# OpenGVLab/VisionLLM

Hardware: NVIDIA H100
Metric: img_text_pairs_per_sec_fwd_1024px_256tok (higher is better)
Workload: dtype bf16

## Files before the change

include/vllm_b200.h:

```cpp
#ifndef VLLM_B200_H
#define VLLM_B200_H
#include <stdint.h>
#include <stddef.h>
#ifdef __cplusplus
extern "C" {
#endif

#define VLLM_OK 0
#define VLLM_EINVAL (-1)
#define VLLM_EUNSUPPORTED (-2)
#define VLLM_EALIGN (-3)

const char* vllm_version(void);

#define VLLM_MSDA_STRICT 1
int vllm_msda_forward_f32(const float* value, const int64_t* spatial_shapes, const int64_t* level_start_index,
                          const float* sampling_loc, const float* attn_weight, float* out, int batch,
                          int spatial_size, int num_heads, int channels, int num_levels, int num_query,
                          int num_point, const int64_t* host_shapes_hint, int flags, void* stream);
int vllm_msda_forward_bf16v(const void* value, const int64_t* spatial_shapes, const int64_t* level_start_index,
                            const float* sampling_loc, const float* attn_weight, void* out, int out_bf16, int batch,
                            int spatial_size, int num_heads, int channels, int num_levels, int num_query,
                            int num_point, const int64_t* host_shapes_hint, void* stream);
int vllm_msda_forward_f64(const double* value, const int64_t* spatial_shapes, const int64_t* level_start_index,
// ... 24 lines not shown
                                 int spatial_size, int num_heads, int channels, int num_levels, int num_query, int num_point,
                                 const int64_t* host_shapes_hint, void* stream);

int vllm_dcnv3_forward_f32(const float* input, const float* offset, const float* mask, float* out, int N,
                           int H_in, int W_in, int H_out, int W_out, int group, int group_channels,
                           int kernel_h, int kernel_w, int stride_h, int stride_w, int pad_h, int pad_w,
                           int dilation_h, int dilation_w, float offset_scale, int flags, void* stream);

int vllm_dcnv3_backward_f32(const float* input, const float* offset, const float* mask, const float* grad_output,
                            float* grad_input, float* grad_offset, float* grad_mask, int N, int H_in, int W_in,
                            int H_out, int W_out, int group, int group_channels, int kernel_h, int kernel_w,
                            int stride_h, int stride_w, int pad_h, int pad_w, int dilation_h, int dilation_w,
                            float offset_scale, void* stream);

#define VLLM_ACT_NONE 0
#define VLLM_ACT_GELU 1
#define VLLM_ACT_RELU 2
#define VLLM_ACT_SILU 3
#define VLLM_ACT_SWIGLU 4
#define VLLM_ACT_QUICKGELU 5
int vllm_gemm_bf16(const void* A, int lda, const void* B, int ldb, void* C, int ldc, int M, int N, int K,
                   const void* bias, const void* colscale, const void* residual, int ldr, int act, int out_f32,
                   void* stream);
int vllm_gemm_bf16_rowmask(const void* A, int lda, const void* B, int ldb, void* C, int ldc, int M, int N, int K,
                           const void* bias, const void* colscale, const void* residual, int ldr, int act, int out_f32,
                           const unsigned char* row_keep, void* stream);
int vllm_gemm_set_sm_limit(int all_gemms, int scatter_gemm);
int vllm_conv_rows_bf16(const void* xpad, long long pad_pixels, int channels, int padded_width, int kernel_h,
                        int kernel_w, const void* weight, int ldw, void* out, int ldo, int out_channels,
                        const void* bias, int act, void* stream);
#define VLLM_GEMM_DEFAULT 0
#define VLLM_GEMM_WIDE_TILE 2
#define VLLM_GEMM_NARROW_TILE 3
int vllm_gemm_set_variant(int variant);

int vllm_rmsnorm_bf16(const void* x, long long ldx, const void* weight, void* y, long long ldy, long long rows,
                      int cols, float eps, void* stream);
int vllm_layernorm_bf16(const void* x, long long ldx, const void* weight, const void* bias, void* y, long long ldy,
                        long long rows, int cols, float eps, void* stream);
int vllm_layernorm_gelu_bf16(const void* x, long long ldx, const void* weight, const void* bias, void* y,
                             long long ldy, long long rows, int cols, float eps, void* stream);
int vllm_layernorm_gather_bf16(const void* x, long long ldx, const int64_t* index, long long rows_in, long long rows_out,
                               long long batch, const void* weight, const void* bias, void* y, long long ldy, int cols,
                               float eps, void* stream);
int vllm_layernorm_residual_bf16(const void* x, long long ldx, const void* weight, const void* bias,
                                 const void* residual, long long ldr, void* y, long long ldy, long long rows, int cols,
                                 float eps, void* stream);
int vllm_dcnv3_prep_f32(const void* packed, long long ld, void* offset, void* mask, void* scale, long long rows,
                        int group, int taps, void* stream);
int vllm_dcnv3_blend_bf16(const void* core, const void* xproj, const void* scale, void* out, long long rows,
                          int channels, int group_channels, void* stream);
int vllm_dwconv_nhwc_bf16(const void* x, const void* weight_taps, const void* bias, void* y, int batch, int height,
                          int width, int channels, int kernel, void* stream);
long long vllm_groupnorm_workspace_bytes(int batch, int groups);
int vllm_groupnorm_nhwc_bf16_grid(const void* x, void* y, const void* gamma, const void* beta, int batch, long long h, long long w,
                                  long long x_w_pitch, long long x_image_pitch, int channels, int groups, float eps, int relu,
                                  void* workspace, long long workspace_bytes, void* stream);
int vllm_upsample_add_nhwc_bf16_ex(const void* top, long long top_image_pitch, const void* lateral, void* out, int batch, int in_h,
                                   int in_w, int out_h, int out_w, int channels, int out_pad, void* stream);
int vllm_rope_bf16(void* x, long long ld, const void* cos, const void* sin, long long tokens, int heads,
                   int head_dim, void* stream);

int vllm_attention_bf16(const void* q, const void* k, const void* v, void* o, int batch, int Tq, int Tk,
                        int heads, int kv_heads, int head_dim, long long q_batch_pitch,
                        long long q_token_pitch, long long k_batch_pitch, long long k_token_pitch,
                        long long v_batch_pitch, long long v_token_pitch, long long o_batch_pitch,
// ... 91 lines not shown
```

visionllm_b200/_lib.py:

```python
import contextlib
import ctypes
import os
import threading

_HERE = os.path.dirname(os.path.abspath(__file__))
LIB_PATH = os.path.join(_HERE, "lib", "libvllm_b200.so")

_lock = threading.Lock()
_lib = None
_launches = 0

c_i64p = ctypes.POINTER(ctypes.c_int64)
vp = ctypes.c_void_p
ci = ctypes.c_int
cll = ctypes.c_longlong
cf = ctypes.c_float

_SIGNATURES = {
    "vllm_version": (ctypes.c_char_p, []),
    "vllm_msda_forward_f32": (ci, [vp, vp, vp, vp, vp, vp, ci, ci, ci, ci, ci, ci, ci, vp, ci, vp]),
    "vllm_msda_forward_bf16v": (ci, [vp, vp, vp, vp, vp, vp, ci, ci, ci, ci, ci, ci, ci, ci, vp, vp]),
    "vllm_msda_forward_f64": (ci, [vp, vp, vp, vp, vp, vp, ci, ci, ci, ci, ci, ci, ci, vp]),
    "vllm_msda_backward_f32": (ci, [vp] * 9 + [ci] * 7 + [vp]),
    "vllm_msda_backward_f64": (ci, [vp] * 9 + [ci] * 7 + [vp]),
# ... 35 lines not shown
    "vllm_layernorm_bf16": (ci, [vp, cll, vp, vp, vp, cll, cll, ci, cf, vp]),
    "vllm_layernorm_gelu_bf16": (ci, [vp, cll, vp, vp, vp, cll, cll, ci, cf, vp]),
    "vllm_layernorm_gather_bf16": (ci, [vp, cll, vp, cll, cll, cll, vp, vp, vp, cll, ci, cf, vp]),
    "vllm_layernorm_residual_bf16": (ci, [vp, cll, vp, vp, vp, cll, vp, cll, cll, ci, cf, vp]),
    "vllm_dcnv3_prep_f32": (ci, [vp, cll, vp, vp, vp, cll, ci, ci, vp]),
    "vllm_dcnv3_blend_bf16": (ci, [vp, vp, vp, vp, cll, ci, ci, vp]),
    "vllm_dwconv_nhwc_bf16": (ci, [vp, vp, vp, vp, ci, ci, ci, ci, ci, vp]),
    "vllm_rope_bf16": (ci, [vp, cll, vp, vp, cll, ci, ci, vp]),
    "vllm_groupnorm_workspace_bytes": (cll, [ci, ci]),
    "vllm_upsample_add_nhwc_bf16_ex": (ci, [vp, cll, vp, vp, ci, ci, ci, ci, ci, ci, ci, vp]),
    "vllm_groupnorm_nhwc_bf16_grid": (ci, [vp, vp, vp, vp, ci, cll, cll, cll, cll, ci, ci, cf, ci, vp, cll, vp]),
    "vllm_attention_bf16": (ci, [vp, vp, vp, vp, ci, ci, ci, ci, ci, ci, cll, cll, cll, cll, cll, cll, cll, cll,
                                 vp, vp, vp, vp, ci, ci, cf, vp, cll, vp]),
    "vllm_attention_bf16_tiles": (ci, [vp, vp, vp, vp, ci, ci, ci, ci, ci, ci, cll, cll, cll, cll, cll, cll, cll, cll,
                                       vp, vp, vp, cf, vp, vp, vp]),
    "vllm_attention_mask_tiles": (ci, [vp, cll, ci, ci, vp, vp, vp]),
    "vllm_attention_set_variant": (ci, [ci]),
    "vllm_attention_set_splits": (ci, [ci]),
    "vllm_peer_alloc": (ci, [ctypes.POINTER(vp), ctypes.c_size_t]),
    "vllm_peer_free": (ci, [vp]),
    "vllm_peer_handle_bytes": (ci, []),
    "vllm_peer_export": (ci, [vp, vp]),
    "vllm_peer_open": (ci, [vp, ctypes.POINTER(vp)]),
    "vllm_peer_close": (ci, [vp]),
    "vllm_gemm_bf16_scatter": (ci, [vp, ci, vp, ci, vp, vp, ci, ci, ci, ci, ci, vp]),
    "vllm_tp_reduce_norm_bf16": (ci, [vp, ci, cll, vp, vp, cf, vp, ci, cll, vp, ctypes.c_uint, vp, ci, ci, ci, vp]),
    "vllm_tp_norm_ctas": (ci, [ci]),
    "vllm_tp_wait": (ci, [vp, ctypes.c_uint, vp]),
    "vllm_tp_signal": (ci, [vp, ci, ctypes.c_uint, vp]),
}


MSDA_DEFAULT, MSDA_NO_HINT, MSDA_BF16_NO_WINDOW, MSDA_FP32_WINDOW = 0, 4, 32, 33
GEMM_DEFAULT, GEMM_WIDE_TILE, GEMM_NARROW_TILE = 0, 2, 3
ATTN_DEFAULT, ATTN_WARP_MMA = 0, 1

_KNOB_DEFAULTS = {"msda_set_variant": (MSDA_DEFAULT,), "msda_set_window": (0, 0, 0), "msda_set_window_fill": (-1,),
                  "gemm_set_variant": (GEMM_DEFAULT,), "gemm_set_sm_limit": (0, 0), "attention_set_variant": (ATTN_DEFAULT,),
                  "attention_set_splits": (0,)}


class VllmB200Error(RuntimeError):
    pass


def exported_symbols():
    return sorted(_SIGNATURES)


def lib():
    global _lib
    if _lib is None:
        with _lock:
            if _lib is None:
                if not os.path.exists(LIB_PATH):
                    raise ImportError(
                        f"{LIB_PATH} is missing: build it with `make` or "
                        "`python -c 'import __graft_entry__ as g; g.build()'`. "
                        "visionllm_b200 has no CPU/eager fallback.")
                L = ctypes.CDLL(LIB_PATH)
                for name, (res, args) in _SIGNATURES.items():
                    fn = getattr(L, name)
                    fn.restype = res
                    fn.argtypes = args
                _lib = L
    return _lib

# ... 34 lines not shown
```

visionllm_b200/csrc/gemm.cu:

```cuda
#include "common.cuh"
#include "tc_common.cuh"
#include "vllm_b200.h"

namespace {

constexpr int BM = 128, BK = 64, THREADS = 384, CONSUMER_WARPS = 8, CONSUMER_THREADS = CONSUMER_WARPS * 32;
constexpr int A_BYTES = BM * BK * 2;
constexpr int EPI_BUF = 16 * 128;
constexpr int SMEM_LIMIT = 232448;

enum { ACT_NONE = 0, ACT_GELU = 1, ACT_RELU = 2, ACT_SILU = 3, ACT_SWIGLU = 4, ACT_QUICKGELU = 5 };

struct GemmArgs {
  int M, N, K;
  void* C; int ldc;
  const __nv_bfloat16* bias; const __nv_bfloat16* colscale; const __nv_bfloat16* residual; int ldr;
  int act; int out_f32;
  const unsigned char* row_keep;
  int tiles_m, tiles_n;
  int group_m;
  int a_seg_kb, a_seg_rows;
  int sc_rows;
  void* sc_dst[8];
  uint32_t* sc_flag[8];
  int a_mn, b_mn;
  int bt_rows, causal;
  int group, reduce;
};

struct TilePlan { int skip, kb0, kb1, segs, b_row_off, a_k_off, b_k_off; };
__device__ __forceinline__ TilePlan plan_tile(const GemmArgs& g, int m0, int n0, int rows_per_tile, int num_kb) {
  TilePlan p{0, 0, num_kb, 1, 0, 0, 0};
  if (g.bt_rows) {
    const int bh = m0 / g.bt_rows, ml = m0 - bh * g.bt_rows;
    const int a_mat = g.reduce ? bh * g.group : bh;
    const int b_mat = g.reduce ? bh * g.group : bh / g.group;
    p.segs = g.reduce ? g.group : 1;
    p.b_row_off = b_mat * g.N;
    p.a_k_off = a_mat * g.K;
    p.b_k_off = b_mat * g.K;
    if (g.causal == 1 && n0 >= ml + rows_per_tile) p.skip = 1;
    if (g.causal == 2) p.kb0 = ml / BK;
    if (g.causal == 3) { const int e = (ml + rows_per_tile + BK - 1) / BK; p.kb1 = e < num_kb ? e : num_kb; }
  }
  return p;
}

template <int BN> struct Cfg {
  static constexpr int B_BYTES = BN * BK * 2;
  static constexpr int STAGE_BYTES = A_BYTES + B_BYTES;
  static constexpr int STAGES = BN == 256 ? 4 : 6;
  static constexpr int EPI_OFF = STAGES * STAGE_BYTES;
  static constexpr int BAR_OFF = EPI_OFF + CONSUMER_WARPS * 2 * EPI_BUF;
  static constexpr int BIAS_OFF = BAR_OFF + 256;
  static constexpr int SCALE_OFF = BIAS_OFF + 2 * BN + 4;
  static constexpr int KEEP_OFF = SCALE_OFF + 2 * BN + 4;
  static constexpr int SMEM = 1024  + KEEP_OFF + BM + 4;
  static_assert(8 * (2 * STAGES + 2 * CONSUMER_WARPS) <= 256, "mbarriers overflow their slot");
  static_assert(SMEM <= SMEM_LIMIT, "shared memory over the per-block limit");
};

__device__ __forceinline__ float gelu_erf(float x) { return 0.5f * x * (1.f + erff(x * 0.70710678118654752f)); }
__device__ __forceinline__ float silu(float x) { return x / (1.f + __expf(-x)); }

__device__ __forceinline__ void tile_coords(int t, int tiles_m, int tiles_n, int group_m, int& tm, int& tn) {
  const int per_group = group_m * tiles_n;
  const int group = t / per_group;
  const int first = group * group_m;
  const int gsz = min(group_m, tiles_m - first);
  const int in = t - group * per_group;
  tm = first + in % gsz;
  tn = in / gsz;
}

template <int BN, int TA, int TB>
__device__ __forceinline__ void mma_kblock(float (&acc)[BN / 2], uint32_t sa, uint32_t sb, bool first_kb) {
  const uint64_t adesc = TA ? tc::wgmma_desc_sw128(sa, 8192, 1024) : tc::wgmma_desc_sw128(sa, 16, 1024);
  const uint64_t bdesc = TB ? tc::wgmma_desc_sw128(sb, 8192, 1024) : tc::wgmma_desc_sw128(sb, 16, 1024);
  constexpr uint64_t astep = TA ? 128 : 2, bstep = TB ? 128 : 2;
#pragma unroll
  for (int k = 0; k < BK / 16; ++k) {
    if constexpr (BN == 256)
      tc::wgmma_m64n256k16_ss<TA, TB>(acc, adesc + astep * k, bdesc + bstep * k, !(first_kb && k == 0));
    else
      tc::wgmma_m64n128k16_ss<TA, TB>(acc, adesc + astep * k, bdesc + bstep * k, !(first_kb && k == 0));
  }
}

enum { EPI_BF16 = 0, EPI_SWIGLU = 1, EPI_F32 = 2, EPI_SCATTER = 3 };

__device__ __forceinline__ int swz(int r, int b) { return r * 128 + ((((b >> 4) ^ r) & 7) << 4) + (b & 15); }

template <int BN, int TA, int TB, int EPI>
__global__ void __launch_bounds__(THREADS, 1)
gemm_bf16_wgmma_kernel(const __grid_constant__ CUtensorMap tmap_a, const __grid_constant__ CUtensorMap tmap_b,
                       const __grid_constant__ CUtensorMap tmap_c, const __grid_constant__ CUtensorMap tmap_r,
                       const GemmArgs g) {
  using C_ = Cfg<BN>;
  constexpr int STAGES = C_::STAGES;
  extern __shared__ uint8_t smem_raw[];
  const uint32_t smem_base = (tc::smem_u32(smem_raw) + 1023u) & ~1023u;
  uint8_t* smem_gen = smem_raw + (smem_base - tc::smem_u32(smem_raw));
  const uint32_t bar_base = smem_base + C_::BAR_OFF;
  auto full_bar = [&](int s) { return bar_base + 8 * s; };
  auto empty_bar = [&](int s) { return bar_base + 8 * (STAGES + s); };
  auto res_bar = [&](int i) { return bar_base + 8 * (2 * STAGES + i); };

  const int warp = threadIdx.x >> 5, lane = threadIdx.x & 31;
  const int n_tiles = g.tiles_m * g.tiles_n;
  const int num_kb = (g.K + BK - 1) / BK;

  if (warp == 0 && lane == 0) {
    tc::tma_prefetch_desc(&tmap_a);
    tc::tma_prefetch_desc(&tmap_b);
    if constexpr (EPI != EPI_SCATTER) {
      tc::tma_prefetch_desc(&tmap_c);
      if (g.residual) tc::tma_prefetch_desc(&tmap_r);
    }
  }
  if (warp == 1 && lane == 0) {
    for (int s = 0; s < STAGES; ++s) { tc::mbar_init(full_bar(s), 1); tc::mbar_init(empty_bar(s), CONSUMER_WARPS); }
    for (int i = 0; i < 2 * CONSUMER_WARPS; ++i) tc::mbar_init(res_bar(i), 1);
    tc::mbar_fence_init();
  }
  __syncthreads();

  if (warp < 4) {
    tc::reg_dealloc<40>();
    if (warp == 0 && tc::elect_one()) {
      int stage = 0; uint32_t phase = 0;
      for (int t = blockIdx.x; t < n_tiles; t += gridDim.x) {
        int tm, tn; tile_coords(t, g.tiles_m, g.tiles_n, g.group_m, tm, tn);
        const TilePlan tp = plan_tile(g, tm * BM, tn * BN, BM, num_kb);
        if (tp.skip) continue;
        const int bt_m0 = g.bt_rows ? (tm * BM) / g.bt_rows * g.bt_rows : 0;
        const int row_a = tm * BM - (TA ? bt_m0 : 0);
        const int row_b = tn * BN + (TB ? 0 : tp.b_row_off);
        for (int gs = 0; gs < tp.segs; ++gs) {
          const int ka_off = TA ? tp.a_k_off + gs * g.K : 0, kb_off = TB ? tp.b_k_off + gs * g.K : 0;
          for (int kb = tp.kb0; kb < tp.kb1; ++kb) {
            tc::mbar_wait(empty_bar(stage), phase ^ 1);
            const uint32_t sa = smem_base + stage * C_::STAGE_BYTES, sb = sa + A_BYTES;
            int ka = kb * BK + ka_off, ra = row_a;
            if (g.a_seg_kb) {
              const int seg = kb / g.a_seg_kb;
              ka = (kb - seg * g.a_seg_kb) * BK;
              ra = row_a + seg * g.a_seg_rows;
            }
            tc::mbar_arrive_expect_tx(full_bar(stage), C_::STAGE_BYTES);
            if constexpr (TA) {
              for (int h = 0; h < BM / 64; ++h) tc::tma_load_2d(sa + h * 8192, &tmap_a, full_bar(stage), ra + 64 * h, ka);
            } else {
              tc::tma_load_2d(sa, &tmap_a, full_bar(stage), ka, ra);
            }
            if constexpr (TB) {
              for (int h = 0; h < BN / 64; ++h)
                tc::tma_load_2d(sb + h * 8192, &tmap_b, full_bar(stage), row_b + 64 * h, kb * BK + kb_off);
            } else {
              tc::tma_load_2d(sb, &tmap_b, full_bar(stage), kb * BK, row_b);
            }
            if (++stage == STAGES) { stage = 0; phase ^= 1; }
          }
        }
      }
    }
    return;
  }

  tc::reg_alloc<232>();
  const int wg = (warp - 4) >> 2;
  const int cw = warp - 4;
  const int et = threadIdx.x - 128;
  const int lr = lane >> 2, frag_col = 2 * (lane & 3);
  const bool has_res = EPI != EPI_SCATTER && g.residual != nullptr;
  constexpr int UNIT_COLS = EPI == EPI_SWIGLU ? 128 : 64;
  constexpr int UNITS = BN / UNIT_COLS;
  constexpr int RES_AHEAD = EPI == EPI_F32 ? 1 : 2;
  const int n_out = EPI == EPI_SWIGLU ? g.N / 2 : g.N;
  uint8_t* s_buf = smem_gen + C_::EPI_OFF + cw * 2 * EPI_BUF;
  const uint32_t s_buf_u32 = smem_base + C_::EPI_OFF + cw * 2 * EPI_BUF;
  const uint32_t s_bias = smem_base + C_::BIAS_OFF, s_scale = smem_base + C_::SCALE_OFF, s_keep = smem_base + C_::KEEP_OFF;
  const __nv_bfloat16* bias_t = reinterpret_cast<const __nv_bfloat16*>(smem_gen + C_::BIAS_OFF + (reinterpret_cast<uintptr_t>(g.bias) & 3));
  const __nv_bfloat16* scale_t =
      reinterpret_cast<const __nv_bfloat16*>(smem_gen + C_::SCALE_OFF + (reinterpret_cast<uintptr_t>(g.colscale) & 3));
  const uint8_t* keep_t = smem_gen + C_::KEEP_OFF + (reinterpret_cast<uintptr_t>(g.row_keep) & 3);
  if (et <= BN / 2) {
    if (!g.bias) *reinterpret_cast<uint32_t*>(smem_gen + C_::BIAS_OFF + 4 * et) = 0u;
    if (!g.colscale) *reinterpret_cast<uint32_t*>(smem_gen + C_::SCALE_OFF + 4 * et) = 0x3F803F80u;
  }
  uint32_t res_phase = 0;
  int stage = 0; uint32_t phase = 0;
  float acc[BN / 2];
  for (int t = blockIdx.x; t < n_tiles; t += gridDim.x) {
    int tm, tn; tile_coords(t, g.tiles_m, g.tiles_n, g.group_m, tm, tn);
    const TilePlan tp = plan_tile(g, tm * BM, tn * BN, BM, num_kb);
    if (tp.skip) continue;
    const int n0 = tn * BN;
    const int oc0 = EPI == EPI_SWIGLU ? n0 / 2 : n0;
    const int warp_row0 = tm * BM + cw * 16;
    const bool warp_live = warp_row0 < g.M;
    if (g.bias && et <= BN / 2) tc::cp_async_vec_word(s_bias, g.bias, 2LL * g.N, 2LL * n0, et);
    if (g.colscale && et <= BN / 2) tc::cp_async_vec_word(s_scale, g.colscale, 2LL * g.N, 2LL * n0, et);
    if (g.row_keep && et <= BM / 4) tc::cp_async_vec_word(s_keep, g.row_keep, g.M, (long long)tm * BM, et);
    auto load_res = [&](int u) {
      const int b = EPI == EPI_F32 ? 0 : (u & 1);
      tc::mbar_arrive_expect_tx(res_bar(2 * cw + b), EPI_BUF);
      tc::tma_load_2d(s_buf_u32 + b * EPI_BUF, &tmap_r, res_bar(2 * cw + b), oc0 + 64 * u, warp_row0);
    };
    if (has_res && warp_live && lane == 0) {
      tc::bulk_wait_read<0>();
#pragma unroll
      for (int u = 0; u < RES_AHEAD && u < UNITS; ++u)
        if (oc0 + 64 * u < n_out) load_res(u);
    }
    int prev_stage = -1;
    const int n_kb = tp.segs * (tp.kb1 - tp.kb0);
    for (int kb = 0; kb < n_kb; ++kb) {
      tc::mbar_wait(full_bar(stage), phase);
      const uint32_t sa = smem_base + stage * C_::STAGE_BYTES + wg * 8192, sb = smem_base + stage * C_::STAGE_BYTES + A_BYTES;
      const bool first = kb == 0;
      tc::acc_fence(acc);
      tc::wgmma_fence();
      mma_kblock<BN, TA, TB>(acc, sa, sb, first);
      tc::wgmma_commit();
      tc::wgmma_wait<1>();
      if (prev_stage >= 0 && lane == 0) tc::mbar_arrive(empty_bar(prev_stage));
      prev_stage = stage;
      if (++stage == STAGES) { stage = 0; phase ^= 1; }
    }
    tc::wgmma_wait<0>();
    tc::acc_fence(acc);
    if (lane == 0) tc::mbar_arrive(empty_bar(prev_stage));
    tc::cp_async_wait_all();
    tc::named_bar_sync(1, CONSUMER_THREADS);

#pragma unroll
    for (int j = 0; j < BN / 8; ++j) {
      const int c = 8 * j + frag_col;
      const float b0 = __bfloat162float(bias_t[c]), b1 = __bfloat162float(bias_t[c + 1]);
      acc[4 * j] = __fadd_rn(acc[4 * j], b0); acc[4 * j + 1] = __fadd_rn(acc[4 * j + 1], b1);
      acc[4 * j + 2] = __fadd_rn(acc[4 * j + 2], b0); acc[4 * j + 3] = __fadd_rn(acc[4 * j + 3], b1);
    }
    if constexpr (EPI == EPI_BF16 || EPI == EPI_F32) {
      switch (g.act) {
        case ACT_GELU:
#pragma unroll
          for (int i = 0; i < BN / 2; ++i) acc[i] = gelu_erf(acc[i]);
          break;
        case ACT_RELU:
#pragma unroll
          for (int i = 0; i < BN / 2; ++i) acc[i] = fmaxf(acc[i], 0.f);
          break;
        case ACT_SILU:
#pragma unroll
          for (int i = 0; i < BN / 2; ++i) acc[i] = silu(acc[i]);
          break;
        case ACT_QUICKGELU:
#pragma unroll
          for (int i = 0; i < BN / 2; ++i) acc[i] = acc[i] / (1.f + __expf(-1.702f * acc[i]));
          break;
        default: break;
      }
    }
    bool keep0 = true, keep1 = true;
    if (g.row_keep) { keep0 = keep_t[cw * 16 + lr] != 0; keep1 = keep_t[cw * 16 + lr + 8] != 0; }

    constexpr int E = EPI == EPI_F32 ? 4 : 2;
    auto put_box = [&](int bi, int col0) {
      if ((n_out * E) % 16 == 0 || col0 + 128 / E <= n_out) {
        if (lane == 0) tc::tma_store_2d(&tmap_c, s_buf_u32 + bi * EPI_BUF, col0, warp_row0);
        return;
      }
#pragma unroll
      for (int it = 0; it < 4; ++it) {
        const int rr = it * 4 + (lane >> 3), piece = lane & 7, row = warp_row0 + rr;
        if (row >= g.M) continue;
#pragma unroll
        for (int e = 0; e < 16 / E; ++e) {
          const int col = col0 + piece * (16 / E) + e;
          if (col >= n_out) break;
          const uint8_t* sp = s_buf + bi * EPI_BUF + swz(rr, 16 * piece + E * e);
          uint8_t* dp = reinterpret_cast<uint8_t*>(g.C) + ((size_t)row * g.ldc + col) * E;
          if constexpr (E == 4) *reinterpret_cast<uint32_t*>(dp) = *reinterpret_cast<const uint32_t*>(sp);
          else *reinterpret_cast<uint16_t*>(dp) = *reinterpret_cast<const uint16_t*>(sp);
        }
      }
    };

    if (warp_live) {
#pragma unroll
      for (int u = 0; u < UNITS; ++u) {
        if (oc0 + 64 * u >= n_out) break;
        const int b = EPI == EPI_F32 ? 0 : (u & 1);
        uint8_t* buf = s_buf + b * EPI_BUF;
        if (has_res) {
          if (u > 0 && u + RES_AHEAD - 1 < UNITS && oc0 + 64 * (u + RES_AHEAD - 1) < n_out && lane == 0) {
            tc::bulk_wait_read<0>();
            load_res(u + RES_AHEAD - 1);
          }
          tc::mbar_wait(res_bar(2 * cw + b), (res_phase >> b) & 1);
          res_phase ^= 1u << b;
        } else if constexpr (EPI != EPI_SCATTER && EPI != EPI_F32) {
          if (lane == 0) { if (u == 0) tc::bulk_wait_read<0>(); else tc::bulk_wait_read<1>(); }
          __syncwarp();
        }
        if constexpr (EPI == EPI_SWIGLU) {
#pragma unroll
          for (int jj = 0; jj < 16; ++jj) {
            const int j = 16 * u + jj;
#pragma unroll
            for (int h = 0; h < 2; ++h) {
              uint8_t* p = buf + swz(lr + 8 * h, 16 * (jj >> 1)) + 8 * (jj & 1) + 2 * (lane & 3);
              float o = __fmul_rn(silu(acc[4 * j + 2 * h]), acc[4 * j + 2 * h + 1]);
              if (has_res) o = __fadd_rn(o, __bfloat162float(*reinterpret_cast<const __nv_bfloat16*>(p)));
              *reinterpret_cast<__nv_bfloat16*>(p) = __float2bfloat16(o);
            }
          }
        } else {
#pragma unroll
          for (int jj = 0; jj < 8; ++jj) {
            const int j = 8 * u + jj, c = 8 * j + frag_col;
            const float s0 = __bfloat162float(scale_t[c]), s1 = __bfloat162float(scale_t[c + 1]);
#pragma unroll
            for (int h = 0; h < 2; ++h) {
              float& v0 = acc[4 * j + 2 * h];
              float& v1 = acc[4 * j + 2 * h + 1];
              uint8_t* p = buf + swz(lr + 8 * h, 16 * jj) + 4 * (lane & 3);
              v0 = __fmul_rn(v0, s0); v1 = __fmul_rn(v1, s1);
              if (has_res) {
                const float2 f = __bfloat1622float2(*reinterpret_cast<const __nv_bfloat162*>(p));
                v0 = __fadd_rn(v0, f.x); v1 = __fadd_rn(v1, f.y);
              }
              if (!(h ? keep1 : keep0)) { v0 = 0.f; v1 = 0.f; }
              if constexpr (EPI != EPI_F32) *reinterpret_cast<__nv_bfloat162*>(p) = __floats2bfloat162_rn(v0, v1);
            }
          }
          if constexpr (EPI == EPI_F32) {
            if (lane == 0) tc::bulk_wait_read<0>();
            __syncwarp();
#pragma unroll
            for (int jj = 0; jj < 8; ++jj) {
              const int j = 8 * u + jj;
#pragma unroll
              for (int h = 0; h < 2; ++h) {
                uint8_t* p = s_buf + (jj >> 2) * EPI_BUF + swz(lr + 8 * h, 32 * (jj & 3) + 8 * (lane & 3));
                *reinterpret_cast<float2*>(p) = make_float2(acc[4 * j + 2 * h], acc[4 * j + 2 * h + 1]);
              }
            }
          }
        }
        if constexpr (EPI == EPI_SCATTER) {
          __syncwarp();
          const int d = warp_row0 / g.sc_rows;
          __nv_bfloat16* dst = reinterpret_cast<__nv_bfloat16*>(g.sc_dst[d]) + (size_t)(warp_row0 - d * g.sc_rows) * g.ldc + n0 + 64 * u;
#pragma unroll
          for (int it = 0; it < 4; ++it) {
            const int rr = it * 4 + (lane >> 3), piece = lane & 7;
            const uint4 val = *reinterpret_cast<const uint4*>(buf + swz(rr, 16 * piece));
            *reinterpret_cast<uint4*>(dst + (size_t)rr * g.ldc + piece * 8) = val;
          }
          __syncwarp();
        } else {
          tc::fence_proxy_async_smem();
          __syncwarp();
          if constexpr (EPI == EPI_F32) {
            put_box(0, n0 + 64 * u);
            if (n0 + 64 * u + 32 < n_out) put_box(1, n0 + 64 * u + 32);
          } else {
            put_box(b, oc0 + 64 * u);
          }
          if (lane == 0) tc::bulk_commit();
        }
      }
    }
    if constexpr (EPI == EPI_SCATTER) {
      __threadfence_system();
      __syncwarp();
      if (lane == 0 && warp_live)
        asm volatile("red.release.sys.global.add.u32 [%0], %1;" ::"l"(g.sc_flag[warp_row0 / g.sc_rows]), "r"(1u) : "memory");
    }
    tc::named_bar_sync(1, CONSUMER_THREADS);
  }
  if (EPI != EPI_SCATTER && lane == 0) tc::bulk_wait<0>();
}

int g_sm_limit = 0, g_scatter_sm_limit = 0;

int g_gemm_variant = VLLM_GEMM_DEFAULT;

using KernelFn = void (*)(const CUtensorMap, const CUtensorMap, const CUtensorMap, const CUtensorMap, const GemmArgs);

template <int BN, int TA, int TB>
KernelFn pick_epilogue(const GemmArgs& g) {
  if (g.sc_rows) {
    if constexpr (BN == 256 && !TA && !TB) return gemm_bf16_wgmma_kernel<BN, TA, TB, EPI_SCATTER>;
    return nullptr;
  }
  if (g.act == ACT_SWIGLU) {
    if constexpr (!TA && !TB) return gemm_bf16_wgmma_kernel<BN, TA, TB, EPI_SWIGLU>;
    return nullptr;
  }
  if (g.out_f32) return gemm_bf16_wgmma_kernel<BN, TA, TB, EPI_F32>;
  return gemm_bf16_wgmma_kernel<BN, TA, TB, EPI_BF16>;
}
template <int BN>
KernelFn pick_kernel(const GemmArgs& g) {
  if (g.a_mn) return g.b_mn ? pick_epilogue<BN, 1, 1>(g) : pick_epilogue<BN, 1, 0>(g);
  return g.b_mn ? pick_epilogue<BN, 0, 1>(g) : pick_epilogue<BN, 0, 0>(g);
}

template <int BN>
int launch_gemm(const void* A, int lda, const void* B, int ldb, GemmArgs g, cudaStream_t st, long long a_rows = -1,
                int a_cols = -1) {
  using C_ = Cfg<BN>;
  CUtensorMap ta, tb;
  const uint64_t nb = g.bt_rows ? (uint64_t)(g.M / g.bt_rows) : 1;
  const uint64_t na = g.bt_rows && g.reduce ? nb * g.group : nb;
  const uint64_t nbb = !g.bt_rows ? 1 : g.reduce ? nb * g.group : nb / g.group;
  const uint64_t m_local = g.bt_rows ? (uint64_t)g.bt_rows : (uint64_t)g.M;
  int rc = g.a_mn ? vllm_make_tmap_2d(&ta, A, na * (uint64_t)g.K, m_local, (uint64_t)lda, 64)
                  : vllm_make_tmap_2d(&ta, A, (uint64_t)(a_rows < 0 ? g.M : a_rows),
                                        (uint64_t)(a_cols < 0 ? g.K : a_cols), (uint64_t)lda, BM);
  if (rc) return rc;
  rc = g.b_mn ? vllm_make_tmap_2d(&tb, B, nbb * (uint64_t)g.K, (uint64_t)g.N, (uint64_t)ldb, 64)
              : vllm_make_tmap_2d(&tb, B, nbb * (uint64_t)g.N, (uint64_t)g.K, (uint64_t)ldb, BN);
  if (rc) return rc;
  CUtensorMap tc_{}, tr{};
  if (!g.sc_rows) {
    const uint64_t n_out = (uint64_t)(g.act == ACT_SWIGLU ? g.N / 2 : g.N);
    rc = vllm_make_tmap_2d(&tc_, g.C, (uint64_t)g.M, n_out, (uint64_t)g.ldc, 16, g.out_f32 != 0);
    if (!rc && g.residual) rc = vllm_make_tmap_2d(&tr, g.residual, (uint64_t)g.M, n_out, (uint64_t)g.ldr, 16);
    if (rc) return rc;
  }
  g.tiles_m = (g.M + BM - 1) / BM;
  g.tiles_n = (g.N + BN - 1) / BN;
  const int n_tiles = g.tiles_m * g.tiles_n;
  int sms = vllm_num_sms();
  const int limit = g.sc_rows ? (g_scatter_sm_limit > 0 ? g_scatter_sm_limit : g_sm_limit) : g_sm_limit;
  if (limit > 0 && limit < sms) sms = limit;
  const int ctas = sms < n_tiles ? sms : n_tiles;
  g.group_m = 8;
  const KernelFn kern = pick_kernel<BN>(g);
  if (!kern) return VLLM_EUNSUPPORTED;
  const cudaError_t e = vllm_smem_optin(kern, C_::SMEM);
  if (e != cudaSuccess) return (int)e;
  kern<<<ctas, THREADS, C_::SMEM, st>>>(ta, tb, tc_, tr, g);
  VLLM_CHECK_LAUNCH();
  return VLLM_OK;
}

bool wide_by_shape(const GemmArgs& g) {
  return !g.a_mn && !g.b_mn && !g.bt_rows && !g.a_seg_kb && g.N >= 2048;
}

int launch_gemm_auto(const void* A, int lda, const void* B, int ldb, const GemmArgs& g, cudaStream_t st, long long a_rows = -1,
                     int a_cols = -1) {
  const bool wide = g.sc_rows || g_gemm_variant == VLLM_GEMM_WIDE_TILE ||
                    (g_gemm_variant == VLLM_GEMM_DEFAULT && wide_by_shape(g));
  return wide ? launch_gemm<256>(A, lda, B, ldb, g, st, a_rows, a_cols) : launch_gemm<128>(A, lda, B, ldb, g, st, a_rows, a_cols);
}

}

extern "C" {

int vllm_gemm_set_variant(int v) {
  if (v != VLLM_GEMM_DEFAULT && v != VLLM_GEMM_WIDE_TILE && v != VLLM_GEMM_NARROW_TILE) return VLLM_EINVAL;
  g_gemm_variant = v;
  return VLLM_OK;
}
int vllm_gemm_set_sm_limit(int all_gemms, int scatter_gemm) {
  if (all_gemms < 0 || scatter_gemm < 0) return VLLM_EINVAL;
  g_sm_limit = all_gemms; g_scatter_sm_limit = scatter_gemm;
  return VLLM_OK;
}

static int gemm_bf16_common(const void* A, int lda, const void* B, int ldb, void* C, int ldc, int M, int N, int K,
                            const void* bias, const void* colscale, const void* residual, int ldr, int act, int out_f32,
                            const unsigned char* row_keep, void* stream);

int vllm_gemm_bf16(const void* A, int lda, const void* B, int ldb, void* C, int ldc, int M, int N, int K,
                   const void* bias, const void* colscale, const void* residual, int ldr, int act, int out_f32,
                   void* stream) {
  return gemm_bf16_common(A, lda, B, ldb, C, ldc, M, N, K, bias, colscale, residual, ldr, act, out_f32, nullptr, stream);
}

int vllm_gemm_bf16_rowmask(const void* A, int lda, const void* B, int ldb, void* C, int ldc, int M, int N, int K,
                           const void* bias, const void* colscale, const void* residual, int ldr, int act, int out_f32,
                           const unsigned char* row_keep, void* stream) {
  if (!row_keep || act == ACT_SWIGLU) return VLLM_EINVAL;
  return gemm_bf16_common(A, lda, B, ldb, C, ldc, M, N, K, bias, colscale, residual, ldr, act, out_f32, row_keep, stream);
}

static int gemm_bf16_common(const void* A, int lda, const void* B, int ldb, void* C, int ldc, int M, int N, int K,
                            const void* bias, const void* colscale, const void* residual, int ldr, int act, int out_f32,
                            const unsigned char* row_keep, void* stream) {
  if (M < 0 || N <= 0 || K <= 0 || lda < K || ldb < K) return VLLM_EINVAL;
  if (M == 0) return VLLM_OK;
  if (!A || !B || !C) return VLLM_EINVAL;
  if (act < 0 || act > ACT_QUICKGELU) return VLLM_EINVAL;
// ... 104 lines not shown
```

Baseline: 6.995.

## Add opt-in ping-pong GEMM schedule and widen tile raster group

Adds a ping-pong variant of the WGMMA GEMM kernel. Each consumer warpgroup computes a full 128x128 tile on its own, using two 64-row accumulators, and the two warpgroups alternate mainloops through ordering mbarriers so one group's epilogue overlaps the other's MMAs. Bias, scale and row-keep vectors are duplicated per warpgroup. The variant only runs when selected explicitly, but the raster group size rises from 8 to 16 for every GEMM, which changes L2 reuse patterns.

```diff
diff --git a/include/vllm_b200.h b/include/vllm_b200.h
--- a/include/vllm_b200.h
+++ b/include/vllm_b200.h
@@ -80,6 +80,7 @@
 #define VLLM_GEMM_DEFAULT 0
 #define VLLM_GEMM_WIDE_TILE 2
 #define VLLM_GEMM_NARROW_TILE 3
+#define VLLM_GEMM_PINGPONG 4
 int vllm_gemm_set_variant(int variant);
 
 int vllm_rmsnorm_bf16(const void* x, long long ldx, const void* weight, void* y, long long ldy, long long rows,
diff --git a/visionllm_b200/_lib.py b/visionllm_b200/_lib.py
--- a/visionllm_b200/_lib.py
+++ b/visionllm_b200/_lib.py
@@ -91,7 +91,7 @@
 
 
 MSDA_DEFAULT, MSDA_NO_HINT, MSDA_BF16_NO_WINDOW, MSDA_FP32_WINDOW = 0, 4, 32, 33
-GEMM_DEFAULT, GEMM_WIDE_TILE, GEMM_NARROW_TILE = 0, 2, 3
+GEMM_DEFAULT, GEMM_WIDE_TILE, GEMM_NARROW_TILE, GEMM_PINGPONG = 0, 2, 3, 4
 ATTN_DEFAULT, ATTN_WARP_MMA = 0, 1
 
 _KNOB_DEFAULTS = {"msda_set_variant": (MSDA_DEFAULT,), "msda_set_window": (0, 0, 0), "msda_set_window_fill": (-1,),
diff --git a/visionllm_b200/csrc/gemm.cu b/visionllm_b200/csrc/gemm.cu
--- a/visionllm_b200/csrc/gemm.cu
+++ b/visionllm_b200/csrc/gemm.cu
@@ -46,7 +46,7 @@
   return p;
 }
 
-template <int BN> struct Cfg {
+template <int BN, bool PINGPONG = false> struct Cfg {
   static constexpr int B_BYTES = BN * BK * 2;
   static constexpr int STAGE_BYTES = A_BYTES + B_BYTES;
   static constexpr int STAGES = BN == 256 ? 4 : 6;
@@ -55,8 +55,11 @@
   static constexpr int BIAS_OFF = BAR_OFF + 256;
   static constexpr int SCALE_OFF = BIAS_OFF + 2 * BN + 4;
   static constexpr int KEEP_OFF = SCALE_OFF + 2 * BN + 4;
-  static constexpr int SMEM = 1024  + KEEP_OFF + BM + 4;
-  static_assert(8 * (2 * STAGES + 2 * CONSUMER_WARPS) <= 256, "mbarriers overflow their slot");
+  static constexpr int VEC_BYTES = KEEP_OFF + BM + 4 - BIAS_OFF;
+  static constexpr int SMEM = 1024  + BIAS_OFF + (PINGPONG ? 2 : 1) * VEC_BYTES;
+  static_assert(!PINGPONG || BN == 128, "the ping-pong schedule runs 128 x 128 tiles");
+  static_assert(VEC_BYTES % 4 == 0, "cp.async words of the second vector set must stay aligned");
+  static_assert(8 * (2 * STAGES + 2 * CONSUMER_WARPS + 2) <= 256, "mbarriers overflow their slot");
   static_assert(SMEM <= SMEM_LIMIT, "shared memory over the per-block limit");
 };
 
@@ -73,17 +76,23 @@
   tn = in / gsz;
 }
 
-template <int BN, int TA, int TB>
-__device__ __forceinline__ void mma_kblock(float (&acc)[BN / 2], uint32_t sa, uint32_t sb, bool first_kb) {
-  const uint64_t adesc = TA ? tc::wgmma_desc_sw128(sa, 8192, 1024) : tc::wgmma_desc_sw128(sa, 16, 1024);
+template <int BN, int TA, int TB, int RB>
+__device__ __forceinline__ void mma_kblock(float (&acc)[RB][BN / 2], uint32_t sa, uint32_t sb, bool first_kb) {
+  uint64_t adesc[RB];
+#pragma unroll
+  for (int rb = 0; rb < RB; ++rb)
+    adesc[rb] = TA ? tc::wgmma_desc_sw128(sa + 8192 * rb, 8192, 1024) : tc::wgmma_desc_sw128(sa + 8192 * rb, 16, 1024);
   const uint64_t bdesc = TB ? tc::wgmma_desc_sw128(sb, 8192, 1024) : tc::wgmma_desc_sw128(sb, 16, 1024);
   constexpr uint64_t astep = TA ? 128 : 2, bstep = TB ? 128 : 2;
 #pragma unroll
   for (int k = 0; k < BK / 16; ++k) {
-    if constexpr (BN == 256)
-      tc::wgmma_m64n256k16_ss<TA, TB>(acc, adesc + astep * k, bdesc + bstep * k, !(first_kb && k == 0));
-    else
-      tc::wgmma_m64n128k16_ss<TA, TB>(acc, adesc + astep * k, bdesc + bstep * k, !(first_kb && k == 0));
+#pragma unroll
+    for (int rb = 0; rb < RB; ++rb) {
+      if constexpr (BN == 256)
+        tc::wgmma_m64n256k16_ss<TA, TB>(acc[rb], adesc[rb] + astep * k, bdesc + bstep * k, !(first_kb && k == 0));
+      else
+        tc::wgmma_m64n128k16_ss<TA, TB>(acc[rb], adesc[rb] + astep * k, bdesc + bstep * k, !(first_kb && k == 0));
+    }
   }
 }
 
@@ -91,13 +100,16 @@
 
 __device__ __forceinline__ int swz(int r, int b) { return r * 128 + ((((b >> 4) ^ r) & 7) << 4) + (b & 15); }
 
-template <int BN, int TA, int TB, int EPI>
+template <int BN, int TA, int TB, int EPI, bool PINGPONG = false>
 __global__ void __launch_bounds__(THREADS, 1)
 gemm_bf16_wgmma_kernel(const __grid_constant__ CUtensorMap tmap_a, const __grid_constant__ CUtensorMap tmap_b,
                        const __grid_constant__ CUtensorMap tmap_c, const __grid_constant__ CUtensorMap tmap_r,
                        const GemmArgs g) {
-  using C_ = Cfg<BN>;
+  static_assert(!PINGPONG || (!TA && !TB && EPI != EPI_SCATTER), "ping-pong serves dense K-major forward launches");
+  using C_ = Cfg<BN, PINGPONG>;
   constexpr int STAGES = C_::STAGES;
+  constexpr int RB = PINGPONG ? 2 : 1;
+  constexpr int TILE_THREADS = PINGPONG ? 128 : CONSUMER_THREADS;
   extern __shared__ uint8_t smem_raw[];
   const uint32_t smem_base = (tc::smem_u32(smem_raw) + 1023u) & ~1023u;
   uint8_t* smem_gen = smem_raw + (smem_base - tc::smem_u32(smem_raw));
@@ -105,6 +117,7 @@
   auto full_bar = [&](int s) { return bar_base + 8 * s; };
   auto empty_bar = [&](int s) { return bar_base + 8 * (STAGES + s); };
   auto res_bar = [&](int i) { return bar_base + 8 * (2 * STAGES + i); };
+  auto order_bar = [&](int w) { return bar_base + 8 * (2 * STAGES + 2 * CONSUMER_WARPS + w); };
 
   const int warp = threadIdx.x >> 5, lane = threadIdx.x & 31;
   const int n_tiles = g.tiles_m * g.tiles_n;
@@ -119,8 +132,9 @@
     }
   }
   if (warp == 1 && lane == 0) {
-    for (int s = 0; s < STAGES; ++s) { tc::mbar_init(full_bar(s), 1); tc::mbar_init(empty_bar(s), CONSUMER_WARPS); }
+    for (int s = 0; s < STAGES; ++s) { tc::mbar_init(full_bar(s), 1); tc::mbar_init(empty_bar(s), TILE_THREADS / 32); }
     for (int i = 0; i < 2 * CONSUMER_WARPS; ++i) tc::mbar_init(res_bar(i), 1);
+    if constexpr (PINGPONG) { tc::mbar_init(order_bar(0), 4); tc::mbar_init(order_bar(1), 4); }
     tc::mbar_fence_init();
   }
   __syncthreads();
@@ -170,7 +184,8 @@
   tc::reg_alloc<232>();
   const int wg = (warp - 4) >> 2;
   const int cw = warp - 4;
-  const int et = threadIdx.x - 128;
+  const int wrow = PINGPONG ? 16 * (cw & 3) : 16 * cw;
+  const int et = threadIdx.x - 128 - (PINGPONG ? 128 * wg : 0);
   const int lr = lane >> 2, frag_col = 2 * (lane & 3);
   const bool has_res = EPI != EPI_SCATTER && g.residual != nullptr;
   constexpr int UNIT_COLS = EPI == EPI_SWIGLU ? 128 : 64;
@@ -179,101 +194,135 @@
   const int n_out = EPI == EPI_SWIGLU ? g.N / 2 : g.N;
   uint8_t* s_buf = smem_gen + C_::EPI_OFF + cw * 2 * EPI_BUF;
   const uint32_t s_buf_u32 = smem_base + C_::EPI_OFF + cw * 2 * EPI_BUF;
-  const uint32_t s_bias = smem_base + C_::BIAS_OFF, s_scale = smem_base + C_::SCALE_OFF, s_keep = smem_base + C_::KEEP_OFF;
-  const __nv_bfloat16* bias_t = reinterpret_cast<const __nv_bfloat16*>(smem_gen + C_::BIAS_OFF + (reinterpret_cast<uintptr_t>(g.bias) & 3));
+  const int vec = PINGPONG ? wg * C_::VEC_BYTES : 0;
+  const uint32_t s_bias = smem_base + C_::BIAS_OFF + vec, s_scale = smem_base + C_::SCALE_OFF + vec,
+                 s_keep = smem_base + C_::KEEP_OFF + vec;
+  const __nv_bfloat16* bias_t =
+      reinterpret_cast<const __nv_bfloat16*>(smem_gen + C_::BIAS_OFF + vec + (reinterpret_cast<uintptr_t>(g.bias) & 3));
   const __nv_bfloat16* scale_t =
-      reinterpret_cast<const __nv_bfloat16*>(smem_gen + C_::SCALE_OFF + (reinterpret_cast<uintptr_t>(g.colscale) & 3));
-  const uint8_t* keep_t = smem_gen + C_::KEEP_OFF + (reinterpret_cast<uintptr_t>(g.row_keep) & 3);
+      reinterpret_cast<const __nv_bfloat16*>(smem_gen + C_::SCALE_OFF + vec + (reinterpret_cast<uintptr_t>(g.colscale) & 3));
+  const uint8_t* keep_t = smem_gen + C_::KEEP_OFF + vec + (reinterpret_cast<uintptr_t>(g.row_keep) & 3);
   if (et <= BN / 2) {
-    if (!g.bias) *reinterpret_cast<uint32_t*>(smem_gen + C_::BIAS_OFF + 4 * et) = 0u;
-    if (!g.colscale) *reinterpret_cast<uint32_t*>(smem_gen + C_::SCALE_OFF + 4 * et) = 0x3F803F80u;
+    if (!g.bias) *reinterpret_cast<uint32_t*>(smem_gen + C_::BIAS_OFF + vec + 4 * et) = 0u;
+    if (!g.colscale) *reinterpret_cast<uint32_t*>(smem_gen + C_::SCALE_OFF + vec + 4 * et) = 0x3F803F80u;
   }
   uint32_t res_phase = 0;
   int stage = 0; uint32_t phase = 0;
-  float acc[BN / 2];
-  for (int t = blockIdx.x; t < n_tiles; t += gridDim.x) {
+  auto skip_kblocks = [&](int n) { stage += n; phase ^= (stage / STAGES) & 1; stage %= STAGES; };
+  uint32_t order_phase = wg ? 0 : 1;
+  if (PINGPONG && wg) skip_kblocks(num_kb);
+  float acc[RB][BN / 2];
+  for (int t = blockIdx.x + (PINGPONG ? wg * gridDim.x : 0); t < n_tiles; t += (PINGPONG ? 2 : 1) * gridDim.x) {
     int tm, tn; tile_coords(t, g.tiles_m, g.tiles_n, g.group_m, tm, tn);
     const TilePlan tp = plan_tile(g, tm * BM, tn * BN, BM, num_kb);
     if (tp.skip) continue;
     const int n0 = tn * BN;
     const int oc0 = EPI == EPI_SWIGLU ? n0 / 2 : n0;
-    const int warp_row0 = tm * BM + cw * 16;
-    const bool warp_live = warp_row0 < g.M;
+    const int row0 = tm * BM + wrow;
+    int live_rb = 0;
+#pragma unroll
+    for (int rb = 0; rb < RB; ++rb) live_rb += row0 + 64 * rb < g.M;
+    const int nu = min(UNITS, (n_out - oc0 + 63) / 64);
+    const int n_units = live_rb * nu;
     if (g.bias && et <= BN / 2) tc::cp_async_vec_word(s_bias, g.bias, 2LL * g.N, 2LL * n0, et);
     if (g.colscale && et <= BN / 2) tc::cp_async_vec_word(s_scale, g.colscale, 2LL * g.N, 2LL * n0, et);
     if (g.row_keep && et <= BM / 4) tc::cp_async_vec_word(s_keep, g.row_keep, g.M, (long long)tm * BM, et);
-    auto load_res = [&](int u) {
-      const int b = EPI == EPI_F32 ? 0 : (u & 1);
+    auto load_res = [&](int q) {
+      const int rb = RB > 1 && q >= nu ? 1 : 0, u = q - rb * nu;
+      const int b = EPI == EPI_F32 ? 0 : (q & 1);
       tc::mbar_arrive_expect_tx(res_bar(2 * cw + b), EPI_BUF);
-      tc::tma_load_2d(s_buf_u32 + b * EPI_BUF, &tmap_r, res_bar(2 * cw + b), oc0 + 64 * u, warp_row0);
+      tc::tma_load_2d(s_buf_u32 + b * EPI_BUF, &tmap_r, res_bar(2 * cw + b), oc0 + 64 * u, row0 + 64 * rb);
     };
-    if (has_res && warp_live && lane == 0) {
+    if (has_res && n_units > 0 && lane == 0) {
       tc::bulk_wait_read<0>();
 #pragma unroll
-      for (int u = 0; u < RES_AHEAD && u < UNITS; ++u)
-        if (oc0 + 64 * u < n_out) load_res(u);
-    }
+      for (int q = 0; q < RES_AHEAD; ++q)
+        if (q < n_units) load_res(q);
+    }
+    if constexpr (PINGPONG) { tc::mbar_wait(order_bar(wg), order_phase); order_phase ^= 1; }
     int prev_stage = -1;
     const int n_kb = tp.segs * (tp.kb1 - tp.kb0);
     for (int kb = 0; kb < n_kb; ++kb) {
       tc::mbar_wait(full_bar(stage), phase);
-      const uint32_t sa = smem_base + stage * C_::STAGE_BYTES + wg * 8192, sb = smem_base + stage * C_::STAGE_BYTES + A_BYTES;
+      const uint32_t sa = smem_base + stage * C_::STAGE_BYTES + (PINGPONG ? 0 : wg * 8192),
+                     sb = smem_base + stage * C_::STAGE_BYTES + A_BYTES;
       const bool first = kb == 0;
-      tc::acc_fence(acc);
+#pragma unroll
+      for (int rb = 0; rb < RB; ++rb) tc::acc_fence(acc[rb]);
       tc::wgmma_fence();
-      mma_kblock<BN, TA, TB>(acc, sa, sb, first);
+      mma_kblock<BN, TA, TB, RB>(acc, sa, sb, first);
       tc::wgmma_commit();
       tc::wgmma_wait<1>();
       if (prev_stage >= 0 && lane == 0) tc::mbar_arrive(empty_bar(prev_stage));
       prev_stage = stage;
       if (++stage == STAGES) { stage = 0; phase ^= 1; }
     }
+    if constexpr (PINGPONG) {
+      if (lane == 0) tc::mbar_arrive(order_bar(wg ^ 1));
+      skip_kblocks(num_kb);
+    }
     tc::wgmma_wait<0>();
-    tc::acc_fence(acc);
+#pragma unroll
+    for (int rb = 0; rb < RB; ++rb) tc::acc_fence(acc[rb]);
     if (lane == 0) tc::mbar_arrive(empty_bar(prev_stage));
     tc::cp_async_wait_all();
-    tc::named_bar_sync(1, CONSUMER_THREADS);
-
-#pragma unroll
-    for (int j = 0; j < BN / 8; ++j) {
-      const int c = 8 * j + frag_col;
-      const float b0 = __bfloat162float(bias_t[c]), b1 = __bfloat162float(bias_t[c + 1]);
-      acc[4 * j] = __fadd_rn(acc[4 * j], b0); acc[4 * j + 1] = __fadd_rn(acc[4 * j + 1], b1);
-      acc[4 * j + 2] = __fadd_rn(acc[4 * j + 2], b0); acc[4 * j + 3] = __fadd_rn(acc[4 * j + 3], b1);
+    tc::named_bar_sync(PINGPONG ? 2 + wg : 1, TILE_THREADS);
+
+#pragma unroll
+    for (int rb = 0; rb < RB; ++rb) {
+#pragma unroll
+      for (int j = 0; j < BN / 8; ++j) {
+        const int c = 8 * j + frag_col;
+        const float b0 = __bfloat162float(bias_t[c]), b1 = __bfloat162float(bias_t[c + 1]);
+        acc[rb][4 * j] = __fadd_rn(acc[rb][4 * j], b0); acc[rb][4 * j + 1] = __fadd_rn(acc[rb][4 * j + 1], b1);
+        acc[rb][4 * j + 2] = __fadd_rn(acc[rb][4 * j + 2], b0); acc[rb][4 * j + 3] = __fadd_rn(acc[rb][4 * j + 3], b1);
+      }
     }
     if constexpr (EPI == EPI_BF16 || EPI == EPI_F32) {
       switch (g.act) {
         case ACT_GELU:
 #pragma unroll
-          for (int i = 0; i < BN / 2; ++i) acc[i] = gelu_erf(acc[i]);
+          for (int rb = 0; rb < RB; ++rb)
+#pragma unroll
+            for (int i = 0; i < BN / 2; ++i) acc[rb][i] = gelu_erf(acc[rb][i]);
           break;
         case ACT_RELU:
 #pragma unroll
-          for (int i = 0; i < BN / 2; ++i) acc[i] = fmaxf(acc[i], 0.f);
+          for (int rb = 0; rb < RB; ++rb)
+#pragma unroll
+            for (int i = 0; i < BN / 2; ++i) acc[rb][i] = fmaxf(acc[rb][i], 0.f);
           break;
         case ACT_SILU:
 #pragma unroll
-          for (int i = 0; i < BN / 2; ++i) acc[i] = silu(acc[i]);
+          for (int rb = 0; rb < RB; ++rb)
+#pragma unroll
+            for (int i = 0; i < BN / 2; ++i) acc[rb][i] = silu(acc[rb][i]);
           break;
         case ACT_QUICKGELU:
 #pragma unroll
-          for (int i = 0; i < BN / 2; ++i) acc[i] = acc[i] / (1.f + __expf(-1.702f * acc[i]));
+          for (int rb = 0; rb < RB; ++rb)
+#pragma unroll
+            for (int i = 0; i < BN / 2; ++i) acc[rb][i] = acc[rb][i] / (1.f + __expf(-1.702f * acc[rb][i]));
           break;
         default: break;
       }
     }
-    bool keep0 = true, keep1 = true;
-    if (g.row_keep) { keep0 = keep_t[cw * 16 + lr] != 0; keep1 = keep_t[cw * 16 + lr + 8] != 0; }
+    bool keep[RB][2];
+#pragma unroll
+    for (int rb = 0; rb < RB; ++rb) {
+      keep[rb][0] = keep[rb][1] = true;
+      if (g.row_keep) { keep[rb][0] = keep_t[wrow + 64 * rb + lr] != 0; keep[rb][1] = keep_t[wrow + 64 * rb + lr + 8] != 0; }
+    }
 
     constexpr int E = EPI == EPI_F32 ? 4 : 2;
-    auto put_box = [&](int bi, int col0) {
+    auto put_box = [&](int bi, int col0, int r0) {
       if ((n_out * E) % 16 == 0 || col0 + 128 / E <= n_out) {
-        if (lane == 0) tc::tma_store_2d(&tmap_c, s_buf_u32 + bi * EPI_BUF, col0, warp_row0);
+        if (lane == 0) tc::tma_store_2d(&tmap_c, s_buf_u32 + bi * EPI_BUF, col0, r0);
         return;
       }
 #pragma unroll
       for (int it = 0; it < 4; ++it) {
-        const int rr = it * 4 + (lane >> 3), piece = lane & 7, row = warp_row0 + rr;
+        const int rr = it * 4 + (lane >> 3), piece = lane & 7, row = r0 + rr;
         if (row >= g.M) continue;
 #pragma unroll
         for (int e = 0; e < 16 / E; ++e) {
@@ -287,21 +336,26 @@
       }
     };
 
-    if (warp_live) {
+#pragma unroll
+    for (int rb = 0; rb < RB; ++rb) {
+      if (rb >= live_rb) break;
+      const int r0 = row0 + 64 * rb;
 #pragma unroll
       for (int u = 0; u < UNITS; ++u) {
-        if (oc0 + 64 * u >= n_out) break;
-        const int b = EPI == EPI_F32 ? 0 : (u & 1);
+        if (u >= nu) break;
+        const int q = rb * nu + u;
+        const int b = EPI == EPI_F32 ? 0 : (q & 1);
         uint8_t* buf = s_buf + b * EPI_BUF;
         if (has_res) {
-          if (u > 0 && u + RES_AHEAD - 1 < UNITS && oc0 + 64 * (u + RES_AHEAD - 1) < n_out && lane == 0) {
+          if constexpr (RB > 1) __syncwarp();
+          if (q > 0 && q + RES_AHEAD - 1 < n_units && lane == 0) {
             tc::bulk_wait_read<0>();
-            load_res(u + RES_AHEAD - 1);
+            load_res(q + RES_AHEAD - 1);
           }
           tc::mbar_wait(res_bar(2 * cw + b), (res_phase >> b) & 1);
           res_phase ^= 1u << b;
         } else if constexpr (EPI != EPI_SCATTER && EPI != EPI_F32) {
-          if (lane == 0) { if (u == 0) tc::bulk_wait_read<0>(); else tc::bulk_wait_read<1>(); }
+          if (lane == 0) { if (q == 0) tc::bulk_wait_read<0>(); else tc::bulk_wait_read<1>(); }
           __syncwarp();
         }
         if constexpr (EPI == EPI_SWIGLU) {
@@ -311,7 +365,7 @@
 #pragma unroll
             for (int h = 0; h < 2; ++h) {
               uint8_t* p = buf + swz(lr + 8 * h, 16 * (jj >> 1)) + 8 * (jj & 1) + 2 * (lane & 3);
-              float o = __fmul_rn(silu(acc[4 * j + 2 * h]), acc[4 * j + 2 * h + 1]);
+              float o = __fmul_rn(silu(acc[rb][4 * j + 2 * h]), acc[rb][4 * j + 2 * h + 1]);
               if (has_res) o = __fadd_rn(o, __bfloat162float(*reinterpret_cast<const __nv_bfloat16*>(p)));
               *reinterpret_cast<__nv_bfloat16*>(p) = __float2bfloat16(o);
             }
@@ -323,15 +377,15 @@
             const float s0 = __bfloat162float(scale_t[c]), s1 = __bfloat162float(scale_t[c + 1]);
 #pragma unroll
             for (int h = 0; h < 2; ++h) {
-              float& v0 = acc[4 * j + 2 * h];
-              float& v1 = acc[4 * j + 2 * h + 1];
+              float& v0 = acc[rb][4 * j + 2 * h];
+              float& v1 = acc[rb][4 * j + 2 * h + 1];
               uint8_t* p = buf + swz(lr + 8 * h, 16 * jj) + 4 * (lane & 3);
               v0 = __fmul_rn(v0, s0); v1 = __fmul_rn(v1, s1);
               if (has_res) {
                 const float2 f = __bfloat1622float2(*reinterpret_cast<const __nv_bfloat162*>(p));
                 v0 = __fadd_rn(v0, f.x); v1 = __fadd_rn(v1, f.y);
               }
-              if (!(h ? keep1 : keep0)) { v0 = 0.f; v1 = 0.f; }
+              if (!keep[rb][h]) { v0 = 0.f; v1 = 0.f; }
               if constexpr (EPI != EPI_F32) *reinterpret_cast<__nv_bfloat162*>(p) = __floats2bfloat162_rn(v0, v1);
             }
           }
@@ -344,15 +398,15 @@
 #pragma unroll
               for (int h = 0; h < 2; ++h) {
                 uint8_t* p = s_buf + (jj >> 2) * EPI_BUF + swz(lr + 8 * h, 32 * (jj & 3) + 8 * (lane & 3));
-                *reinterpret_cast<float2*>(p) = make_float2(acc[4 * j + 2 * h], acc[4 * j + 2 * h + 1]);
+                *reinterpret_cast<float2*>(p) = make_float2(acc[rb][4 * j + 2 * h], acc[rb][4 * j + 2 * h + 1]);
               }
             }
           }
         }
         if constexpr (EPI == EPI_SCATTER) {
           __syncwarp();
-          const int d = warp_row0 / g.sc_rows;
-          __nv_bfloat16* dst = reinterpret_cast<__nv_bfloat16*>(g.sc_dst[d]) + (size_t)(warp_row0 - d * g.sc_rows) * g.ldc + n0 + 64 * u;
+          const int d = r0 / g.sc_rows;
+          __nv_bfloat16* dst = reinterpret_cast<__nv_bfloat16*>(g.sc_dst[d]) + (size_t)(r0 - d * g.sc_rows) * g.ldc + n0 + 64 * u;
 #pragma unroll
           for (int it = 0; it < 4; ++it) {
             const int rr = it * 4 + (lane >> 3), piece = lane & 7;
@@ -364,10 +418,10 @@
           tc::fence_proxy_async_smem();
           __syncwarp();
           if constexpr (EPI == EPI_F32) {
-            put_box(0, n0 + 64 * u);
-            if (n0 + 64 * u + 32 < n_out) put_box(1, n0 + 64 * u + 32);
+            put_box(0, n0 + 64 * u, r0);
+            if (n0 + 64 * u + 32 < n_out) put_box(1, n0 + 64 * u + 32, r0);
           } else {
-            put_box(b, oc0 + 64 * u);
+            put_box(b, oc0 + 64 * u, r0);
           }
           if (lane == 0) tc::bulk_commit();
         }
@@ -376,10 +430,10 @@
     if constexpr (EPI == EPI_SCATTER) {
       __threadfence_system();
       __syncwarp();
-      if (lane == 0 && warp_live)
-        asm volatile("red.release.sys.global.add.u32 [%0], %1;" ::"l"(g.sc_flag[warp_row0 / g.sc_rows]), "r"(1u) : "memory");
-    }
-    tc::named_bar_sync(1, CONSUMER_THREADS);
+      if (lane == 0 && live_rb > 0)
+        asm volatile("red.release.sys.global.add.u32 [%0], %1;" ::"l"(g.sc_flag[row0 / g.sc_rows]), "r"(1u) : "memory");
+    }
+    tc::named_bar_sync(PINGPONG ? 2 + wg : 1, TILE_THREADS);
   }
   if (EPI != EPI_SCATTER && lane == 0) tc::bulk_wait<0>();
 }
@@ -390,29 +444,33 @@
 
 using KernelFn = void (*)(const CUtensorMap, const CUtensorMap, const CUtensorMap, const CUtensorMap, const GemmArgs);
 
-template <int BN, int TA, int TB>
+template <int BN, int TA, int TB, bool PINGPONG>
 KernelFn pick_epilogue(const GemmArgs& g) {
   if (g.sc_rows) {
     if constexpr (BN == 256 && !TA && !TB) return gemm_bf16_wgmma_kernel<BN, TA, TB, EPI_SCATTER>;
     return nullptr;
   }
   if (g.act == ACT_SWIGLU) {
-    if constexpr (!TA && !TB) return gemm_bf16_wgmma_kernel<BN, TA, TB, EPI_SWIGLU>;
+    if constexpr (!TA && !TB) return gemm_bf16_wgmma_kernel<BN, TA, TB, EPI_SWIGLU, PINGPONG>;
     return nullptr;
   }
-  if (g.out_f32) return gemm_bf16_wgmma_kernel<BN, TA, TB, EPI_F32>;
-  return gemm_bf16_wgmma_kernel<BN, TA, TB, EPI_BF16>;
-}
-template <int BN>
+  if (g.out_f32) return gemm_bf16_wgmma_kernel<BN, TA, TB, EPI_F32, PINGPONG>;
+  return gemm_bf16_wgmma_kernel<BN, TA, TB, EPI_BF16, PINGPONG>;
+}
+template <int BN, bool PINGPONG>
 KernelFn pick_kernel(const GemmArgs& g) {
-  if (g.a_mn) return g.b_mn ? pick_epilogue<BN, 1, 1>(g) : pick_epilogue<BN, 1, 0>(g);
-  return g.b_mn ? pick_epilogue<BN, 0, 1>(g) : pick_epilogue<BN, 0, 0>(g);
-}
-
-template <int BN>
+  if constexpr (PINGPONG) {
+    return pick_epilogue<BN, 0, 0, true>(g);
+  } else {
+    if (g.a_mn) return g.b_mn ? pick_epilogue<BN, 1, 1, false>(g) : pick_epilogue<BN, 1, 0, false>(g);
+    return g.b_mn ? pick_epilogue<BN, 0, 1, false>(g) : pick_epilogue<BN, 0, 0, false>(g);
+  }
+}
+
+template <int BN, bool PINGPONG = false>
 int launch_gemm(const void* A, int lda, const void* B, int ldb, GemmArgs g, cudaStream_t st, long long a_rows = -1,
                 int a_cols = -1) {
-  using C_ = Cfg<BN>;
+  using C_ = Cfg<BN, PINGPONG>;
   CUtensorMap ta, tb;
   const uint64_t nb = g.bt_rows ? (uint64_t)(g.M / g.bt_rows) : 1;
   const uint64_t na = g.bt_rows && g.reduce ? nb * g.group : nb;
@@ -439,8 +497,8 @@
   const int limit = g.sc_rows ? (g_scatter_sm_limit > 0 ? g_scatter_sm_limit : g_sm_limit) : g_sm_limit;
   if (limit > 0 && limit < sms) sms = limit;
   const int ctas = sms < n_tiles ? sms : n_tiles;
-  g.group_m = 8;
-  const KernelFn kern = pick_kernel<BN>(g);
+  g.group_m = 16;
+  const KernelFn kern = pick_kernel<BN, PINGPONG>(g);
   if (!kern) return VLLM_EUNSUPPORTED;
   const cudaError_t e = vllm_smem_optin(kern, C_::SMEM);
   if (e != cudaSuccess) return (int)e;
@@ -449,15 +507,26 @@
   return VLLM_OK;
 }
 
-bool wide_by_shape(const GemmArgs& g) {
-  return !g.a_mn && !g.b_mn && !g.bt_rows && !g.a_seg_kb && g.N >= 2048;
+bool pingpong_ok(const GemmArgs& g) { return !g.a_mn && !g.b_mn && !g.bt_rows && !g.a_seg_kb && !g.sc_rows; }
+
+enum Sched { SCHED_COOP_128, SCHED_COOP_256, SCHED_PINGPONG };
+
+Sched schedule_by_shape(const GemmArgs& g) {
+  if (g.sc_rows) return SCHED_COOP_256;
+  return pingpong_ok(g) && g.N >= 2048 ? SCHED_COOP_256 : SCHED_COOP_128;
 }
 
 int launch_gemm_auto(const void* A, int lda, const void* B, int ldb, const GemmArgs& g, cudaStream_t st, long long a_rows = -1,
                      int a_cols = -1) {
-  const bool wide = g.sc_rows || g_gemm_variant == VLLM_GEMM_WIDE_TILE ||
-                    (g_gemm_variant == VLLM_GEMM_DEFAULT && wide_by_shape(g));
-  return wide ? launch_gemm<256>(A, lda, B, ldb, g, st, a_rows, a_cols) : launch_gemm<128>(A, lda, B, ldb, g, st, a_rows, a_cols);
+  Sched s = schedule_by_shape(g);
+  if (!g.sc_rows && g_gemm_variant == VLLM_GEMM_WIDE_TILE) s = SCHED_COOP_256;
+  if (!g.sc_rows && g_gemm_variant == VLLM_GEMM_NARROW_TILE) s = SCHED_COOP_128;
+  if (!g.sc_rows && g_gemm_variant == VLLM_GEMM_PINGPONG) s = pingpong_ok(g) ? SCHED_PINGPONG : SCHED_COOP_128;
+  switch (s) {
+    case SCHED_COOP_256: return launch_gemm<256>(A, lda, B, ldb, g, st, a_rows, a_cols);
+    case SCHED_PINGPONG: return launch_gemm<128, true>(A, lda, B, ldb, g, st, a_rows, a_cols);
+    default: return launch_gemm<128>(A, lda, B, ldb, g, st, a_rows, a_cols);
+  }
 }
 
 }
@@ -465,7 +534,8 @@
 extern "C" {
 
 int vllm_gemm_set_variant(int v) {
-  if (v != VLLM_GEMM_DEFAULT && v != VLLM_GEMM_WIDE_TILE && v != VLLM_GEMM_NARROW_TILE) return VLLM_EINVAL;
+  if (v != VLLM_GEMM_DEFAULT && v != VLLM_GEMM_WIDE_TILE && v != VLLM_GEMM_NARROW_TILE && v != VLLM_GEMM_PINGPONG)
+    return VLLM_EINVAL;
   g_gemm_variant = v;
   return VLLM_OK;
 }
```

Measured after the change: 7.036 (median of 6 runs). About the same (+0.6%).
